# RohitMovva/VexAutonomousPlanner

Hardware: AMD Instinct MI355X
Metric: trajectory sample-points/sec (batched paths) (higher is better)
Workload: dtype f32; 1 GPU; c3: 4096 paths x 32 waypoints x 10000 samples per GPU; waypoints=32, samples=10000, recurrence=f64 behind fp32 rows, parallelism=paths sharded x1, no data-path collective

## Files before the change

### include/vap.h

```cpp
#ifndef VAP_H
#define VAP_H

#include <stddef.h>
#include <stdint.h>

#ifdef __cplusplus
extern "C" {
#endif

#define VAP_VERSION 100

typedef enum {
    VAP_OK = 0,
    VAP_ERR_INVALID = -1,
    VAP_ERR_NO_DEVICE = -2,
    VAP_ERR_HIP = -3,
    VAP_ERR_UNFITTED = -4,
    VAP_ERR_CAPACITY = -5,
    VAP_ERR_UNSUPPORTED = -6
} vap_status;

typedef enum { VAP_F32 = 0, VAP_F64 = 1 } vap_dtype;

typedef struct {
// ... 10 lines not shown
#define VAP_LUT_SAMPLES 1000
#define VAP_SAMPLES_PER_NODE 1000

typedef struct vap_ctx vap_ctx;

int vap_version(void);
const char *vap_status_string(int status);
const char *vap_last_error(void);
int vap_device_count(void);
int vap_ctx_create(int device, vap_ctx **out);
int vap_ctx_destroy(vap_ctx *ctx);
#define VAP_STREAM_OWN ((void *)(intptr_t)-1)
int vap_ctx_set_stream(vap_ctx *ctx, void *hip_stream);
int vap_ctx_synchronize(vap_ctx *ctx);
enum { VAP_OPT_VELOCITY_KERNEL = 0, VAP_OPT_F32_RECURRENCE = 1,
       VAP_OPT_TIME_DOMAIN_RESIDUAL = 3, VAP_OPT_TIME_KERNEL = 4, VAP_OPT_FOOTPRINT_CULL = 5 };
enum { VAP_VELOCITY_AUTO = 0, VAP_VELOCITY_SEQ_LITERAL = 1, VAP_VELOCITY_SEQ_FAST = 2, VAP_VELOCITY_RELAX = 3,
       VAP_VELOCITY_RELAX_BLOCK = 4 , VAP_VELOCITY_RELAX_WAVE = 5 ,
       VAP_VELOCITY_LANES = 6 , VAP_VELOCITY_LANES_16 = 7, VAP_VELOCITY_LANES_32 = 8,
       VAP_VELOCITY_LANES_64 = 9, VAP_VELOCITY_RELAX_ROUNDS = 10  };
enum { VAP_RECURRENCE_F64 = 0, VAP_RECURRENCE_F32 = 1 };
enum { VAP_TIME_KERNEL_AUTO = 0, VAP_TIME_KERNEL_LANE = 1, VAP_TIME_KERNEL_QUAD = 2, VAP_TIME_KERNEL_FUSED = 3 };
int vap_ctx_set_option(vap_ctx *ctx, int option, int value);
int vap_ctx_set_timing(vap_ctx *ctx, int enabled);
int vap_last_timing(vap_ctx *ctx, float ms[VAP_T_COUNT]);


int vap_fit(vap_ctx *ctx, vap_dtype dt, int B, int W, const void *d_waypoints,
            const double *d_tangent_in, const double *d_tangent_out, double *d_segments,
            double *d_segment_lengths , double *d_meta,
            uint32_t *d_flags);

int vap_fit_ex(vap_ctx *ctx, vap_dtype dt, int B, int W, const void *d_waypoints,
               const double *d_tangent_in, const double *d_tangent_out, const double *d_first_derivatives,
               const double *d_second_derivatives, const double *d_starting_tangent,
               const double *d_ending_tangent, double *d_segments, double *d_segment_lengths,
               double *d_first_out, double *d_second_out, double *d_meta, uint32_t *d_flags);
// ... 136 lines not shown
```

### vexautonomousplanner_amd/_lib.py

```python
import ctypes as C
import os

HERE = os.path.dirname(os.path.abspath(__file__))
LIB_PATH = os.path.join(HERE, "libvap.so")

VAP_OK = 0
VAP_ERR_INVALID = -1
VAP_ERR_NO_DEVICE = -2
VAP_ERR_HIP = -3
VAP_ERR_UNFITTED = -4
VAP_ERR_CAPACITY = -5
VAP_ERR_UNSUPPORTED = -6
VAP_F32 = 0
VAP_F64 = 1
FLAG_DEGENERATE = 1
FLAG_TRUNCATED = 2
FLAG_NOCONVERGE = 4
FLAG_BAD_ROUTE = 8
T_FIT, T_LUT, T_SAMPLE, T_VELOCITY, T_TOTAL, T_COUNT = 0, 1, 2, 3, 4, 8
OPT_VELOCITY_KERNEL = 0
OPT_TIME_DOMAIN_RESIDUAL = 3
OPT_F32_RECURRENCE = 1
OPT_TIME_KERNEL = 4
OPT_FOOTPRINT_CULL = 5
TIME_KERNEL_AUTO, TIME_KERNEL_LANE, TIME_KERNEL_QUAD, TIME_KERNEL_FUSED = 0, 1, 2, 3
RECURRENCE_F64, RECURRENCE_F32 = 0, 1
VELOCITY_AUTO, VELOCITY_SEQ_LITERAL, VELOCITY_SEQ_FAST, VELOCITY_RELAX = 0, 1, 2, 3
VELOCITY_RELAX_BLOCK, VELOCITY_RELAX_WAVE = 4, 5
VELOCITY_LANES, VELOCITY_LANES_16, VELOCITY_LANES_32, VELOCITY_LANES_64 = 6, 7, 8, 9
VELOCITY_RELAX_ROUNDS = 10
LUT_SAMPLES = 1000
SAMPLES_PER_NODE = 1000
CLOSEST_GUI, CLOSEST_EXACT = 0, 1
CLOSEST_MODES = {"gui": CLOSEST_GUI, "exact": CLOSEST_EXACT}


def closest_mode(mode):
    if mode in (CLOSEST_GUI, CLOSEST_EXACT) and not isinstance(mode, bool):
        return int(mode)
# ... 193 lines not shown
```

### vexautonomousplanner_amd/batch.py

```python
import ctypes as C

import numpy as np
import torch

from . import _lib
from .synth import DEFAULT_CONSTRAINTS, END_VEL, START_VEL

FIELDS = ("x", "y", "heading", "curvature", "velocity")


def _torch_dtype(dtype):
    if dtype in ("f32", "fp32", torch.float32, np.float32, _lib.VAP_F32):
        return torch.float32, _lib.VAP_F32
    if dtype in ("f64", "fp64", torch.float64, np.float64, _lib.VAP_F64):
        return torch.float64, _lib.VAP_F64
    raise ValueError(f"unsupported dtype {dtype!r}")


class ProfileResult(dict):
    generation = None


class BatchedTrajectoryGenerator:

# ... 8 lines not shown
        self._L = _lib.lib()
        self.set_velocity_kernel(velocity_kernel)
        self.set_recurrence(recurrence)
        self.time_domain_residual = bool(time_domain_residual)
        self.ctx.set_option(_lib.OPT_TIME_DOMAIN_RESIDUAL, 1 if self.time_domain_residual else 0)
        self._generation = 0

    def set_recurrence(self, which):
        self.recurrence = {"f64": "f64", "f32": "f32", "fp64": "f64", "fp32": "f32"}[which]
        self.ctx.set_option(_lib.OPT_F32_RECURRENCE,
                            _lib.RECURRENCE_F64 if self.recurrence == "f64" else _lib.RECURRENCE_F32)

    def set_time_kernel(self, which):
        self.ctx.set_option(_lib.OPT_TIME_KERNEL, {"auto": _lib.TIME_KERNEL_AUTO, "lane": _lib.TIME_KERNEL_LANE,
                                                   "quad": _lib.TIME_KERNEL_QUAD, "fused": _lib.TIME_KERNEL_FUSED}[which])

    def set_velocity_kernel(self, which):
        table = {"auto": _lib.VELOCITY_AUTO, "seq_literal": _lib.VELOCITY_SEQ_LITERAL,
                 "seq_fast": _lib.VELOCITY_SEQ_FAST, "relax": _lib.VELOCITY_RELAX,
                 "relax_block": _lib.VELOCITY_RELAX_BLOCK, "relax_wave": _lib.VELOCITY_RELAX_WAVE,
                 "lanes": _lib.VELOCITY_LANES, "lanes16": _lib.VELOCITY_LANES_16, "lanes32": _lib.VELOCITY_LANES_32,
                 "lanes64": _lib.VELOCITY_LANES_64, "relax_rounds": _lib.VELOCITY_RELAX_ROUNDS}
        self.ctx.set_option(_lib.OPT_VELOCITY_KERNEL, table[which])

    def profile(self, waypoints, constraints=DEFAULT_CONSTRAINTS, samples=None, dd=None,
                start_vel=START_VEL, end_vel=END_VEL, want=FIELDS, out=None, capacity=None):
        if (samples is None) == (dd is None):
            raise ValueError("give exactly one of samples= or dd=")
        wp = waypoints
        if wp.device != self.device or wp.dtype != self.tdtype or wp.dim() != 3 or wp.shape[2] != 2:
# ... 289 lines not shown
```

### vexautonomousplanner_amd/csrc/vap_api.hip

```cpp
#include <cstdlib>
#include <cstring>

#include "vap_internal.h"
#include "vap_kernels.h"

namespace {
thread_local std::string g_last_error;
}

int vap_fail(int status, const char *fmt, ...)
{
    char buf[512];
    va_list ap;
    va_start(ap, fmt);
    vsnprintf(buf, sizeof(buf), fmt, ap);
    va_end(ap);
    g_last_error = buf;
    return status;
}

int vap_set_device(vap_ctx *ctx)
{
    if (!ctx) return vap_fail(VAP_ERR_INVALID, "null context");
    HIP_TRY(hipSetDevice(ctx->device));
// ... 232 lines not shown
        return VAP_OK;
    }
    if (option == VAP_OPT_TIME_DOMAIN_RESIDUAL && (value == 0 || value == 1)) {
        ctx->keep_residual = value;
        ctx->vres_for = nullptr;
        return VAP_OK;
    }
    if (option == VAP_OPT_TIME_KERNEL && value >= VAP_TIME_KERNEL_AUTO && value <= VAP_TIME_KERNEL_FUSED) {
        ctx->time_kernel = value;
        return VAP_OK;
    }
    if (option == VAP_OPT_FOOTPRINT_CULL && (value == 0 || value == 1)) {
        ctx->footprint_cull = value;
        return VAP_OK;
    }
    if (option == VAP_OPT_F32_RECURRENCE && (value == VAP_RECURRENCE_F64 || value == VAP_RECURRENCE_F32)) {
        ctx->f32_recurrence = value;
        ctx->rows_valid = false;
        return VAP_OK;
    }
    return vap_fail(VAP_ERR_INVALID, "unknown option %d / value %d", option, value);
}

int vap_ctx_set_timing(vap_ctx *ctx, int enabled)
{
    if (!ctx) return vap_fail(VAP_ERR_INVALID, "null context");
    ctx->timing = enabled != 0;
    return VAP_OK;
}

int vap_last_timing(vap_ctx *ctx, float ms[VAP_T_COUNT])
{
    VAP_TRY(vap_set_device(ctx));
    if (!ms) return vap_fail(VAP_ERR_INVALID, "null output");
    for (int i = 0; i < VAP_T_COUNT; i++) ms[i] = 0.f;
    if (!ctx->timing) return VAP_OK;
    HIP_TRY(hipEventSynchronize(ctx->ev[VAP_T_VELOCITY + 1]));
    float total = 0.f;
    for (int i = 0; i <= VAP_T_VELOCITY; i++) {
        float t = 0.f;
        HIP_TRY(hipEventElapsedTime(&t, ctx->ev[i], ctx->ev[i + 1]));
        ms[i] = t;
        total += t;
    }
    ms[VAP_T_TOTAL] = total;
    return VAP_OK;
}

int vap_fit(vap_ctx *ctx, vap_dtype dt, int B, int W, const void *d_waypoints, const double *d_tangent_in,
            const double *d_tangent_out, double *d_segments, double *d_segment_lengths, double *d_meta,
            uint32_t *d_flags)
{
    VAP_TRY(vap_set_device(ctx));
    VAP_TRY(check_shape(B, W, 2));
    if (!d_waypoints || !d_segments || !d_meta) return vap_fail(VAP_ERR_INVALID, "null buffer");
    HIP_TRY(vap::launch_fit(ctx->stream, dt == VAP_F64, B, W, d_waypoints, d_tangent_in, d_tangent_out,
                            d_segments, nullptr, d_segment_lengths, d_meta, d_flags));
    return VAP_OK;
// ... 139 lines not shown
        VAP_TRY(ctx->ensure(ctx->flags, (size_t)B * sizeof(uint32_t)));
        flags = (uint32_t *)ctx->flags.ptr;
    }
    void *curv = d_curvature;
    if (!curv && !hi) {
        VAP_TRY(ctx->ensure(ctx->io[7], n_pts * esz(dt)));
        curv = ctx->io[7].ptr;
    }
    const double cc[6] = {c->max_vel, c->max_acc, c->max_acc, c->friction_coef, c->max_jerk, c->track_width};
    StageTimer tm(ctx);
    vap::GridArgs grid;
    grid.S = S;
    grid.dd = dd;
    grid.aux = (double *)ctx->aux.ptr;
    grid.runs = (double *)ctx->runs.ptr;
    if (vap::fit_lut_fusable(B, W)) {
        tm.mark(VAP_T_FIT);
        HIP_TRY(vap::launch_fit_lut(ctx->stream, f64, B, W, d_waypoints, (double *)ctx->seg.ptr, (double *)ctx->power.ptr,
                                    (double *)ctx->lut.ptr, meta, flags, grid));
    } else {
        HIP_TRY(vap::launch_fit(ctx->stream, f64, B, W, d_waypoints, nullptr, nullptr, (double *)ctx->seg.ptr,
                                (double *)ctx->power.ptr, nullptr, meta, flags));
        tm.mark(VAP_T_FIT);
        HIP_TRY(vap::launch_lut(ctx->stream, B, W, (const double *)ctx->seg.ptr, (double *)ctx->lut.ptr,
                                nullptr, meta, flags, grid));
    }
    tm.mark(VAP_T_LUT);
    {
        HIP_TRY(vap::launch_sample(ctx->stream, f64, B, W, S, (const double *)ctx->power.ptr, (const double *)ctx->lut.ptr, nullptr,
                                   meta, (const double *)ctx->aux.ptr, (const double *)ctx->runs.ptr, d_x, d_y, d_heading,
                                   curv, hi ? nullptr : ctx->dth.ptr, hi ? (double *)ctx->k64.ptr : nullptr,
                                   hi ? (double *)ctx->dth64.ptr : nullptr, (const double *)ctx->seg.ptr));
        tm.mark(VAP_T_SAMPLE);
        if (hi)
            VAP_TRY(run_velocity(ctx, true, false, B, S, cc, start_vel, end_vel, meta, ctx->k64.ptr, ctx->dth64.ptr, nullptr,
                                 vap::AccRowsV(), d_velocity, flags));
        else
            VAP_TRY(run_velocity(ctx, f64, f64, B, S, cc, start_vel, end_vel, meta, curv, ctx->dth.ptr, nullptr, vap::AccRowsV(),
                                 d_velocity, flags));
    }
    tm.mark(VAP_T_VELOCITY);
    ctx->last_B = B;
    ctx->last_W = W;
    ctx->grid_B = B;
    ctx->grid_W = W;
    ctx->grid_S = S;
    ctx->rows_valid = true;
// ... 46 lines not shown
    }
    void *curv = d_curvature;
    if (!curv && !hi) {
        VAP_TRY(ctx->ensure(ctx->io[7], n_pts * esz(dt)));
        curv = ctx->io[7].ptr;
    }
    const double cc[6] = {c->max_vel, c->max_acc, c->max_acc, c->friction_coef, c->max_jerk, c->track_width};
    vap::RouteSplitInputs in;
    in.rev = d_node_reverse;
    in.turn = d_node_turn;
    in.tangent = d_node_tangent;
    in.mag = d_node_magnitudes;
    double *sptab = (double *)ctx->sptab.ptr;
    int *nspl = (int *)ctx->nspl.ptr;
    StageTimer tm(ctx);
    HIP_TRY(vap::launch_fit_routes(ctx->stream, f64, B, W, NS, d_waypoints, in, (double *)ctx->seg.ptr, (double *)ctx->power.ptr,
                                   nullptr, sptab, nspl, meta, flags));
    tm.mark(VAP_T_FIT);
    vap::RouteTables rt;
    rt.sptab = sptab;
    rt.nspl = nspl;
    rt.NS = NS;
    const bool single = NS == 1;
    HIP_TRY(vap::launch_lut(ctx->stream, B, W, (const double *)ctx->seg.ptr, (double *)ctx->lut.ptr, nullptr, meta, flags,
                            vap::GridArgs(), rt));
    HIP_TRY(vap::launch_route_offsets(ctx->stream, B, W, NS, S, dd, (const double *)ctx->lut.ptr, sptab, nspl, meta,
                                      (double *)ctx->aux.ptr, (double *)ctx->runs.ptr, flags));
    tm.mark(VAP_T_LUT);
    if (single)
        HIP_TRY(vap::launch_sample(ctx->stream, f64, B, W, S, (const double *)ctx->power.ptr, (const double *)ctx->lut.ptr,
// ... 298 lines not shown
```

### vexautonomousplanner_amd/csrc/vap_internal.h

```cpp
#pragma once
#include "../../include/vap.h"

#include <hip/hip_runtime.h>

#include <cstdarg>
#include <cstdio>
#include <string>

int vap_fail(int status, const char *fmt, ...);

#define HIP_TRY(expr)                                                                              \
    do {                                                                                           \
        hipError_t e_ = (expr);                                                                    \
        if (e_ != hipSuccess)                                                                      \
            return vap_fail(VAP_ERR_HIP, "%s failed: %s (%s:%d)", #expr, hipGetErrorString(e_), __FILE__, __LINE__); \
    } while (0)

#define VAP_TRY(expr)            \
    do {                         \
        int s_ = (expr);         \
        if (s_ != VAP_OK) return s_; \
    } while (0)

struct VapBuffer {
// ... 5 lines not shown
    int device = 0;
    hipStream_t own_stream = nullptr;
    hipStream_t stream = nullptr;
    bool timing = false;
    int velocity_kernel = 0;
    int f32_recurrence = 0;
    hipEvent_t ev[VAP_T_COUNT + 1] = {};
    float ms[VAP_T_COUNT] = {};
    VapBuffer seg, power, lut, slopes, aux, runs, meta, dth, flags, io[8], small_in, small_out, small_seg, small_lut;
    VapBuffer ufwd, lstate, lcount;
    VapBuffer vhi, vres;
    const void *vres_for = nullptr;
    int vres_B = 0, vres_S = 0;
    int keep_residual = 1;
    int time_kernel = 0;
    VapBuffer k64, dth64;
    VapBuffer sptab, nspl;
    int route_NS = 0;
    int last_B = 0, last_W = 0;
    int grid_B = 0, grid_W = 0, grid_S = 0;
    bool rows_valid = false, rows_hi = false;
    int rows_dt = 0;
    int footprint_cull = 1;
    VapBuffer scene;
    void *scene_host = nullptr;
    size_t scene_host_cap = 0;
    hipEvent_t scene_ev = nullptr;

    int ensure(VapBuffer &b, size_t bytes)
    {
// ... 16 lines not shown
```

### vexautonomousplanner_amd/csrc/vap_kernels.h

```cpp
#pragma once
#include <hip/hip_runtime.h>
#include <stdint.h>

namespace vap {

constexpr uint32_t VAP_FLAG_DEGENERATE_BIT = 1u;
constexpr uint32_t VAP_FLAG_TRUNCATED_BIT = 2u;
constexpr uint32_t VAP_FLAG_NOCONVERGE_BIT = 4u;

constexpr int kSampleThreads = 256;
constexpr int kSPT = 4;
constexpr int kSampleChunk = kSampleThreads * kSPT;
constexpr int kSampleTile = kSampleChunk - kSPT;
constexpr int kCoefBlockDoubles = 36;
constexpr int kGridRunBlockDoubles = 3 * 100;
constexpr int kLdsCoefSegments = 112;
constexpr int kMaxWaypoints = 2048;
constexpr int kMaxRouteWaypoints = 1500;

struct RouteTables {
    const double *sptab = nullptr;
    const int *nspl = nullptr;
    int NS = 1;
};
struct RouteSplitInputs {
    const int *rev = nullptr;
    const double *turn = nullptr;
    const double *tangent = nullptr;
    const double *mag = nullptr;
};
hipError_t launch_fit(hipStream_t st, bool f64, int B, int W, const void *wp, const double *tin,
// ... 9 lines not shown
hipError_t launch_lut(hipStream_t st, int B, int W, const double *seg, double *lut, double *slopes, double *meta,
                      uint32_t *flags, GridArgs grid = GridArgs(), RouteTables rt = RouteTables());
bool fit_lut_fusable(int B, int W);
hipError_t launch_fit_lut(hipStream_t st, bool f64, int B, int W, const void *wp, double *seg, double *pw, double *lut,
                          double *meta, uint32_t *flags, GridArgs grid);
hipError_t launch_fit_routes(hipStream_t st, bool f64, int B, int W, int NS, const void *wp, const RouteSplitInputs &in, double *seg,
                             double *pw, double *seglen, double *sptab, int *nspl, double *meta, uint32_t *flags);
hipError_t launch_route_offsets(hipStream_t st, int B, int W, int NS, int S, double dd, const double *lut, double *sptab,
                                const int *nspl, double *meta, double *aux, double *runs, uint32_t *flags);
hipError_t launch_sample_routes(hipStream_t st, bool f64, int B, int W, int NS, int S, const double *pw, const double *lut,
                                const double *sptab, const int *nspl, const double *meta, const double *aux, const double *runs,
                                void *x, void *y, void *h, void *k, void *dth, double *k64, double *dth64, const double *seg);
hipError_t launch_lut_slopes(hipStream_t st, int B, const double *lut, const double *meta, double *slopes);
hipError_t launch_grid(hipStream_t st, int B, int W, int S, double dd, double *meta, double *aux, double *runs,
                       uint32_t *flags);
hipError_t launch_sample(hipStream_t st, bool f64, int B, int W, int S, const double *pw, const double *lut,
                         const double *slopes, const double *meta, const double *aux, const double *runs, void *x,
                         void *y, void *h, void *k, void *dth, double *k64, double *dth64,
                         const double *seg);
struct AccRowsV {
    const void *fwd = nullptr;
    const void *bwd = nullptr;
    const void *dec = nullptr;
};
hipError_t launch_velocity_seq(hipStream_t st, bool r64, bool io64, bool fast, int B, int S, const double c[6], double sv,
                               double ev, const double *meta, const void *curv, const void *dth, const void *vcap,
                               const AccRowsV &acc, void *vel, void *usq);
int velocity_relax_max_samples(bool f64, bool limits = false);
int velocity_relax_acc_max_samples(bool f64);
hipError_t launch_velocity_relax(hipStream_t st, bool r64, bool io64, int B, int S, const double c[6], double sv, double ev,
                                 const double *meta, const void *curv, const void *dth, const void *vcap,
                                 const AccRowsV &acc, void *vel, uint32_t *flags, void *vhi = nullptr);
size_t velocity_long_state_bytes(bool f64, int B, int S);
size_t velocity_long_counter_bytes(bool f64, int B, int S);
// ... 65 lines not shown
```

### vexautonomousplanner_amd/csrc/vap_kernels.hip

```cpp
#include "vap_device.h"
#include "vap_kernels.h"

#include <cstdio>
#include <cstdlib>
#include <type_traits>
#include <vector>

namespace vap {

static_assert(kCoefBlockDoubles == kCoefDoubles, "scratch sizing and block layout disagree");
static_assert(kGridRunBlockDoubles == kGridRunDoubles, "scratch sizing and run-table layout disagree");

struct FitExtras {
    const double *first = nullptr, *second = nullptr;
    const double *start_tan = nullptr, *end_tan = nullptr;
    double *out_first = nullptr, *out_second = nullptr;
};

template <typename IT>
__device__ __forceinline__ void fit_path(int b, int W, const IT *__restrict__ waypoints, const double *__restrict__ tan_in,
                                         const double *__restrict__ tan_out, const FitExtras &ex, double *__restrict__ segments,
                                         double *__restrict__ power, double *__restrict__ seglen, double *__restrict__ meta,
                                         uint32_t *__restrict__ flags, double *sh, int tid = threadIdx.x, int nt = blockDim.x,
                                         uint32_t *flag_word = nullptr)
// ... 134 lines not shown
    int b = blockIdx.x * per + sub;
    b = b < B ? b : B - 1;
    fit_path<IT>(b, W, waypoints, nullptr, nullptr, FitExtras(), segments, power, nullptr, meta, flags, sh + (size_t)sub * 7 * W, lane, L,
                 &s_flags[sub]);
}

__global__ void k_grid(int B, int W, int S, double dd_in, double *__restrict__ meta, double *__restrict__ aux,
                       double *__restrict__ runs, uint32_t *__restrict__ flags)
{
    const int b = blockIdx.x * blockDim.x + threadIdx.x;
    if (b >= B) return;
    grid_define(b, W, S, dd_in, meta[(size_t)b * kMetaStride + 1], meta[(size_t)b * kMetaStride + 0], meta, aux, runs, flags);
}

constexpr int kLutPad = (kLutN + 31) / 32 * 32;
template <bool SEG_LDS>
__device__ __forceinline__ void lut_path(int W, const double *__restrict__ segments, double *__restrict__ lut,
                                         double *__restrict__ slopes, double *__restrict__ meta, uint32_t *__restrict__ flags,
                                         const GridArgs &grid, const RouteTables &rt, long long *__restrict__ stats, double *s_seg,
                                         double *cum)
{
    const long long tl0 = stats ? __builtin_amdgcn_s_memtime() : 0;
    constexpr int kPad = kLutPad;
    double *mag = cum;
    const int b = blockIdx.x, tid = threadIdx.x, nt = blockDim.x;
    int G = W - 1;
    double t_max;
    const double *seg = segments + (size_t)b * (W - 1) * 12;
    size_t row = (size_t)b;
    if (rt.sptab) {
// ... 32 lines not shown
        for (int it = 0; it < kPer; it++) {
            const int j = tid + it * nt;
            inc[it] = (j > 0 && j < kLutN) ? (mag[j - 1] + mag[j]) * 0.5 * dt : 0.0;
        }
        __syncthreads();
#pragma unroll
        for (int it = 0; it < kPer; it++) {
            const int j = tid + it * nt;
            if (j < kPad) cum[j] = inc[it];
        }
    }
    __syncthreads();
    __shared__ double s_start[kPad / 32];
    __shared__ double s_total;
    if (tid == 0) {
        double acc = 0.0;
        const double2 *cum2 = reinterpret_cast<const double2 *>(cum);
#pragma unroll 1
        for (int g0 = 0; g0 < kPad / 32; g0++) {
            s_start[g0] = acc;
            double2 v[16];
#pragma unroll
            for (int k = 0; k < 16; k++) v[k] = cum2[g0 * 16 + k];
#pragma unroll
            for (int k = 0; k < 16; k++) { acc += v[k].x; acc += v[k].y; }
        }
        if (!rt.sptab) meta[(size_t)b * kMetaStride + 1] = acc;
        s_total = acc;
        if (flags && !(acc > 0.0 && isfinite(acc))) atomicOr(&flags[b], VAP_FLAG_DEGENERATE_BIT);
    }
    __syncthreads();
    if (grid.aux && !rt.sptab && tid == nt - 1) grid_define(b, W, grid.S, grid.dd, s_total, t_max, meta, grid.aux, grid.runs, flags);
    if (tid < kPad / 32) {
        double acc = s_start[tid];
        double2 *cum2 = reinterpret_cast<double2 *>(cum) + tid * 16;
        double2 v[16];
#pragma unroll
        for (int k = 0; k < 16; k++) v[k] = cum2[k];
#pragma unroll
        for (int k = 0; k < 16; k++) {
            acc += v[k].x;
            v[k].x = acc;
            acc += v[k].y;
            v[k].y = acc;
        }
#pragma unroll
        for (int k = 0; k < 16; k++) cum2[k] = v[k];
    }
    __syncthreads();
    const long long tl2 = stats ? __builtin_amdgcn_s_memtime() : 0;
    const double lstep = t_max / (double)(kLutN - 1);
    for (int j = tid; j < kLutN; j += nt) {
        lut[row * kLutN + j] = cum[j];
        if (slopes) {
            double w = 0.0;
            if (j > 0) {
                const double t0 = (double)(j - 1) * lstep, t1 = (j == kLutN - 1) ? t_max : (double)j * lstep;
                w = div_inrange(t1 - t0, cum[j] - cum[j - 1]);
            }
            slopes[row * kLutN + j] = w;
        }
    }
    if (stats && tid == 0) {
// ... 169 lines not shown
                             double *__restrict__ slopes)
{
    const int i = blockIdx.x * blockDim.x + threadIdx.x;
    if (i >= B * kLutN) return;
    const int b = i / kLutN, j = i % kLutN;
    const double t_max = meta[(size_t)b * kMetaStride + 0];
    const double lstep = t_max / (double)(kLutN - 1);
    double w = 0.0;
    if (j > 0) {
        const double t0 = (double)(j - 1) * lstep, t1 = (j == kLutN - 1) ? t_max : (double)j * lstep;
        w = div_inrange(t1 - t0, lut[i] - lut[i - 1]);
    }
    slopes[i] = w;
}

template <typename OT, bool COEF_LDS, bool HI, int PPB = 1>
__global__ __launch_bounds__(kSampleThreads, 3) void k_sample(int B, int W, int S, int tile, int tiles_per_block,
                                                           const double *__restrict__ power,
                                                           const double *__restrict__ seg_rows,
                                                           const double *__restrict__ lut,
                                                           const double *__restrict__ slopes,
                                                           const double *__restrict__ meta,
                                                           const double *__restrict__ aux,
                                                           const double *__restrict__ runs,
                                                           OT *__restrict__ ox, OT *__restrict__ oy,
                                                           OT *__restrict__ oh, OT *__restrict__ ok,
                                                           OT *__restrict__ odth, double *__restrict__ ok64,
                                                           double *__restrict__ odth64, long long *__restrict__ stats)
{
    static_assert(!HI || sizeof(OT) == 4, "the fp64 side rows belong to the fp32 output mode");
    extern __shared__ __attribute__((aligned(16))) double s_coef[];
    __shared__ double sD_all[PPB * kLutN], sWt_all[PPB * kLutN];
    __shared__ double s_dx[2][kSampleThreads], s_dy[2][kSampleThreads];
    __shared__ int s_j[2][kSampleThreads];
    __shared__ OT s_th[2][kSampleThreads];
    const long long ts0 = stats ? __builtin_amdgcn_s_memtime() : 0;
    const int tid = threadIdx.x;
    const int G = W - 1;
    const int tile0 = blockIdx.x * tiles_per_block;
    if (tile0 * tile >= S) return;
    const bool writer = tile == kSampleChunk || tid < kSampleThreads - 1;
    constexpr int VW = 16 / sizeof(OT);
    const bool aligned = (S % VW) == 0;

    int p_b[PPB], p_N[PPB], p_nruns[PPB];
    bool p_live[PPB];
    double p_tmax[PPB], p_total[PPB], p_dd[PPB], p_lstep[PPB], p_tstep[PPB], p_inv[PPB], p_sk[PPB];
    double run_touch = 0.0;
#pragma unroll
    for (int pp = 0; pp < PPB; pp++) {
        const int bq = blockIdx.y * PPB + pp;
        p_live[pp] = bq < B;
        const int b = p_live[pp] ? bq : B - 1;
        p_b[pp] = b;
        const double *m = meta + (size_t)b * kMetaStride;
        p_tmax[pp] = m[0]; p_total[pp] = m[1]; p_dd[pp] = m[2];
        p_N[pp] = (int)m[3];
        const double *ax = aux + (size_t)b * kAuxStride;
        p_lstep[pp] = ax[0]; p_tstep[pp] = ax[1]; p_inv[pp] = ax[2];
        p_nruns[pp] = (int)ax[3];
        run_touch += runs[(size_t)b * kGridRunDoubles + (tid < 120 ? tid : 0)];
    }
    __shared__ double s_end[PPB][2];
    double end_d1x = 1.0, end_d1y = 1.0;
    {
        const int pp = tid < PPB ? tid : 0;
        if (seg_rows && tid < PPB && p_live[pp]) {
            end_d1x = seg_rows[((size_t)p_b[pp] * G + (G - 1)) * 12 + 6];
            end_d1y = seg_rows[((size_t)p_b[pp] * G + (G - 1)) * 12 + 7];
        }
    }
    {
        constexpr int ITER = 4;
        double vD[PPB][ITER], vW[PPB][ITER];
#pragma unroll
        for (int pp = 0; pp < PPB; pp++) {
            const bool go = p_live[pp];
#pragma unroll
// ... 20 lines not shown
                if (p_live[pp])
                    lds_fill<4>(s_coef + (size_t)pp * G * kCoefDoubles, power + (size_t)p_b[pp] * G * kCoefDoubles, G * kCoefDoubles, tid,
                                kSampleThreads);
        }
#pragma unroll
        for (int pp = 0; pp < PPB; pp++) {
#pragma unroll
            for (int it = 0; it < ITER; it++) {
                const int i = tid + it * kSampleThreads;
                if (i < kLutN) {
                    sD_all[pp * kLutN + i] = vD[pp][it];
                    if (slopes) sWt_all[pp * kLutN + i] = vW[pp][it];
                }
            }
        }
    }
    auto grid_first_of = [&](const double *run_tab, double dd, int N, int n_runs, int kb0) {
        const int dd_exp = (__double2hiint(dd) >> 20) & 0x7ff;
        const int kf = kb0 < N - 1 ? kb0 : N - 1;
        int r = 2 + 2 * (((__double2hiint((double)kf * dd) >> 20) & 0x7ff) - dd_exp);
        r = kf <= 0 ? 0 : r < 1 ? 1 : r;
        r = r > n_runs - 1 ? n_runs - 1 : r;
        const double *e = run_tab + 3 * r;
        int ka = (int)grid_run_k0(e, 0);
        const int kb = (int)grid_run_k0(e, 1);
        double sa = e[1], da = e[2];
        if (kf < ka || kf >= kb) {
            while ((int)grid_run_k0(run_tab, r + 1) <= kf) r++;
            while (r > 0 && (int)grid_run_k0(run_tab, r) > kf) r--;
            ka = (int)grid_run_k0(run_tab, r);
            sa = run_tab[3 * r + 1];
            da = run_tab[3 * r + 2];
        }
        return sa + (double)(kf - ka) * da;
    };
#pragma unroll
    for (int pp = 0; pp < PPB; pp++)
        p_sk[pp] = (p_live[pp] && tile0 * tile < p_N[pp])
                       ? grid_first_of(runs + (size_t)p_b[pp] * kGridRunDoubles, p_dd[pp], p_N[pp], p_nruns[pp], tile0 * tile + tid * kSPT)
                       : 0.0;
    constexpr bool kSlopeOnDemand = PPB == 2;
    if (!slopes && !kSlopeOnDemand) {
        __syncthreads();
#pragma unroll
        for (int pp = 0; pp < PPB; pp++) {
            if (p_live[pp] && tile0 * tile < p_N[pp]) {
                const double *sDp = sD_all + pp * kLutN;
                for (int j = tid; j < kLutN; j += kSampleThreads) {
                    double w = 0.0;
                    if (j > 0) {
                        const double t0 = (double)(j - 1) * p_lstep[pp], t1 = (j == kLutN - 1) ? p_tmax[pp] : (double)j * p_lstep[pp];
                        w = div_inrange(t1 - t0, sDp[j] - sDp[j - 1]);
                    }
                    sWt_all[pp * kLutN + j] = w;
                }
            }
        }
    }
    __syncthreads();
    asm volatile("" ::"v"(run_touch));
    const long long ts1 = stats ? __builtin_amdgcn_s_memtime() : 0;
    const double end_param = (double)(W - 1);
    const int tab_n = W * kSamplesPerNode;
    int tiles_done = 0;

#pragma unroll 1
    for (int pp = 0; pp < PPB; pp++) {
    const int bq = blockIdx.y * PPB + pp;
    if (bq >= B) break;
    const int b = bq;
    const double *m = meta + (size_t)b * kMetaStride;
    const double t_max = m[0], total = m[1], dd = m[2];
    const int N = (int)m[3];
    const double *ax = aux + (size_t)b * kAuxStride;
    const double lstep = ax[0], tstep = ax[1], inv_tstep = ax[2];
    const int n_runs = (int)ax[3];
    const size_t row = (size_t)b * S;
    const double *sD = sD_all + pp * kLutN, *sWt = sWt_all + pp * kLutN;
    const double *pw = power + (size_t)b * G * kCoefDoubles;
    const double *coef = COEF_LDS ? s_coef + (size_t)pp * G * kCoefDoubles : pw;
    const double *run_tab = runs + (size_t)b * kGridRunDoubles;
    const double sk_first = PPB == 1 ? p_sk[0] : (pp == 0 ? p_sk[0] : p_sk[PPB - 1]);
    auto grid_first = [&](int kb0) { return grid_first_of(run_tab, dd, N, n_runs, kb0); };
    for (int tl = 0; tl < tiles_per_block; tl++) {
        const int k0 = (tile0 + tl) * tile;
        if (k0 >= S) break;
        const int kbase = k0 + tid * kSPT;
        auto store_vec = [&](OT *dst, const OT v[kSPT]) {
            if (!dst || !writer) return;
            if (aligned && kbase + kSPT <= S) {
                if constexpr (sizeof(OT) == 4) {
                    if constexpr (HI) {
                        using f4 = float __attribute__((ext_vector_type(4)));
                        f4 w = {v[0], v[1], v[2], v[3]};
                        __builtin_nontemporal_store(w, reinterpret_cast<f4 *>(dst + row + kbase));
                    } else {
// ... 235 lines not shown
            }
            store_vec(ox, vx); store_vec(oy, vy); store_vec(oh, vh); store_vec(ok, vk);
            if constexpr (HI) store_hi(odth64, vd64);
            store_vec(odth, vd);
        }
            };
        const bool interior = k0 > 0 && k0 + kSampleThreads * kSPT < N - 1 && aligned && (S & 1) == 0 && k0 + kSampleThreads * kSPT <= S;
        if (interior) tile_body(std::true_type{});
        else tile_body(std::false_type{});
    }
    }
    if (stats && (tid & 63) == 0) {
        long long *st = stats + ((size_t)(blockIdx.y * gridDim.x + blockIdx.x) * 4 + (tid >> 6)) * 4;
        st[0] = ts1 - ts0;
        st[1] = __builtin_amdgcn_s_memtime() - ts1;
        st[2] = 0;
        st[3] = 0;
    }
}


template <typename R, typename IO, bool FAST>
__global__ __launch_bounds__(64) void k_velocity_seq(int B, int S, VelConsts<R> c, R start_u, R end_u,
                                                     const double *__restrict__ meta,
                                                     const R *__restrict__ curv, const R *__restrict__ dtheta,
                                                     const R *__restrict__ vcap, AccRows<R> acc, IO *__restrict__ vel,
                                                     R *__restrict__ usq)
{
    const int b = blockIdx.x * blockDim.x + threadIdx.x;
    if (b >= B) return;
    const double *m = meta + (size_t)b * kMetaStride;
    const R twodd = (R)2 * (R)m[2];
// ... 1371 lines not shown
}

hipError_t launch_lut_slopes(hipStream_t st, int B, const double *lut, const double *meta, double *slopes)
{
    hipLaunchKernelGGL(k_lut_slopes, dim3((B * kLutN + 255) / 256), dim3(256), 0, st, B, lut, meta, slopes);
    return hipGetLastError();
}

hipError_t launch_grid(hipStream_t st, int B, int W, int S, double dd, double *meta, double *aux, double *runs,
                       uint32_t *flags)
{
    hipLaunchKernelGGL(k_grid, dim3((B + 63) / 64), dim3(64), 0, st, B, W, S, dd, meta, aux, runs, flags);
    return hipGetLastError();
}

hipError_t launch_sample(hipStream_t st, bool f64, int B, int W, int S, const double *pw, const double *lut,
                         const double *slopes, const double *meta, const double *aux, const double *runs, void *x,
                         void *y, void *h, void *k, void *dth, double *k64, double *dth64, const double *seg)
{
    const bool hi = !f64 && k64 && dth64;
    const int tile = S <= kSampleChunk ? kSampleChunk : kSampleTile;
    const int n_tiles = (S + tile - 1) / tile;
    int split = (2048 + B - 1) / B;
    split = split < 1 ? 1 : (split > n_tiles ? n_tiles : split);
    const int tiles_per_block = (n_tiles + split - 1) / split;
    const bool in_lds = (W - 1) <= kLdsCoefSegments;
    const int ppb = (n_tiles == 1 && B >= 8192 && in_lds && (W - 1) <= 16) ? 2 : 1;
    const dim3 grid((n_tiles + tiles_per_block - 1) / tiles_per_block, (B + ppb - 1) / ppb);
    const size_t lds = in_lds ? sizeof(double) * (size_t)ppb * (W - 1) * kCoefDoubles : 0;
    static const bool want_stats = getenv("VAP_SAMPLE_STATS") != nullptr;
    long long *stats = nullptr;
    const size_t n_waves = (size_t)grid.x * grid.y * 4;
    if (want_stats) (void)hipMalloc(&stats, n_waves * 4 * sizeof(long long));
#define VAP_SAMPLE(OT_, LDS_, HI_, PPB_)                                                                            \
    hipLaunchKernelGGL((k_sample<OT_, LDS_, HI_, PPB_>), grid, dim3(kSampleThreads), lds, st, B, W, S, tile, tiles_per_block, pw, seg, lut, \
                       slopes, meta, aux, runs, (OT_ *)x, (OT_ *)y, (OT_ *)h, (OT_ *)k, (OT_ *)dth, k64, dth64, stats)
    if (ppb == 2) {
        if (f64) VAP_SAMPLE(double, true, false, 2);
        else if (hi) VAP_SAMPLE(float, true, true, 2);
        else VAP_SAMPLE(float, true, false, 2);
    } else if (f64) { if (in_lds) VAP_SAMPLE(double, true, false, 1); else VAP_SAMPLE(double, false, false, 1); }
    else if (hi) { if (in_lds) VAP_SAMPLE(float, true, true, 1); else VAP_SAMPLE(float, false, true, 1); }
    else { if (in_lds) VAP_SAMPLE(float, true, false, 1); else VAP_SAMPLE(float, false, false, 1); }
#undef VAP_SAMPLE
    if (stats) {
        std::vector<long long> h(n_waves * 4);
        (void)hipStreamSynchronize(st);
        (void)hipMemcpy(h.data(), stats, h.size() * sizeof(long long), hipMemcpyDeviceToHost);
        (void)hipFree(stats);
        double sum[4] = {0, 0, 0, 0};
        for (size_t w = 0; w < n_waves; w++)
            for (int k = 0; k < 4; k++) sum[k] += (double)h[w * 4 + k];
        fprintf(stderr, "[sample grid %ux%u, %d tiles/block] per-wave mean ticks: stage %.0f tiles %.0f\n", grid.x,
                grid.y, tiles_per_block, sum[0] / n_waves, sum[1] / n_waves);
    }
    return hipGetLastError();
}

template <typename R>
static VelConsts<R> make_consts(const double c[6])
{
    VelConsts<R> v;
    v.vmax = (R)c[0];
    v.amax = (R)c[1];
    v.adec = (R)c[2];
    v.tw = (R)c[5];
    v.wmax = (R)2 * v.vmax / v.tw;
// ... 348 lines not shown
```

Measured before the change: 46.42 billion sample-points/s.

## Fuse spline fit and arc-length LUT build into the sampling kernel

Adds a FIT variant of the sample kernel in which each workgroup fits its own path's spline, builds the arc-length table and grid runs in LDS, and then samples directly. The separate fit/LUT launch and the global round trip of coefficients, LUT, meta and aux are removed, though the results are still written back to global memory for later stages. On by default when B>=2048, W-1<=48 and one path per block. The cost is serial fit work at the start of every sampling workgroup, higher LDS use that may lower occupancy, and wider template specialisation.

```diff
diff --git a/include/vap.h b/include/vap.h
--- a/include/vap.h
+++ b/include/vap.h
@@ -48,13 +48,14 @@
 int vap_ctx_set_stream(vap_ctx *ctx, void *hip_stream);
 int vap_ctx_synchronize(vap_ctx *ctx);
 enum { VAP_OPT_VELOCITY_KERNEL = 0, VAP_OPT_F32_RECURRENCE = 1,
-       VAP_OPT_TIME_DOMAIN_RESIDUAL = 3, VAP_OPT_TIME_KERNEL = 4, VAP_OPT_FOOTPRINT_CULL = 5 };
+       VAP_OPT_TIME_DOMAIN_RESIDUAL = 3, VAP_OPT_TIME_KERNEL = 4, VAP_OPT_FOOTPRINT_CULL = 5, VAP_OPT_FIT_IN_SAMPLER = 6 };
 enum { VAP_VELOCITY_AUTO = 0, VAP_VELOCITY_SEQ_LITERAL = 1, VAP_VELOCITY_SEQ_FAST = 2, VAP_VELOCITY_RELAX = 3,
        VAP_VELOCITY_RELAX_BLOCK = 4 , VAP_VELOCITY_RELAX_WAVE = 5 ,
        VAP_VELOCITY_LANES = 6 , VAP_VELOCITY_LANES_16 = 7, VAP_VELOCITY_LANES_32 = 8,
        VAP_VELOCITY_LANES_64 = 9, VAP_VELOCITY_RELAX_ROUNDS = 10  };
 enum { VAP_RECURRENCE_F64 = 0, VAP_RECURRENCE_F32 = 1 };
 enum { VAP_TIME_KERNEL_AUTO = 0, VAP_TIME_KERNEL_LANE = 1, VAP_TIME_KERNEL_QUAD = 2, VAP_TIME_KERNEL_FUSED = 3 };
+enum { VAP_FIT_IN_SAMPLER_AUTO = 0, VAP_FIT_IN_SAMPLER_OFF = 1 };
 int vap_ctx_set_option(vap_ctx *ctx, int option, int value);
 int vap_ctx_set_timing(vap_ctx *ctx, int enabled);
 int vap_last_timing(vap_ctx *ctx, float ms[VAP_T_COUNT]);
diff --git a/vexautonomousplanner_amd/_lib.py b/vexautonomousplanner_amd/_lib.py
--- a/vexautonomousplanner_amd/_lib.py
+++ b/vexautonomousplanner_amd/_lib.py
@@ -23,6 +23,8 @@
 OPT_F32_RECURRENCE = 1
 OPT_TIME_KERNEL = 4
 OPT_FOOTPRINT_CULL = 5
+OPT_FIT_IN_SAMPLER = 6
+FIT_IN_SAMPLER_AUTO, FIT_IN_SAMPLER_OFF = 0, 1
 TIME_KERNEL_AUTO, TIME_KERNEL_LANE, TIME_KERNEL_QUAD, TIME_KERNEL_FUSED = 0, 1, 2, 3
 RECURRENCE_F64, RECURRENCE_F32 = 0, 1
 VELOCITY_AUTO, VELOCITY_SEQ_LITERAL, VELOCITY_SEQ_FAST, VELOCITY_RELAX = 0, 1, 2, 3
diff --git a/vexautonomousplanner_amd/batch.py b/vexautonomousplanner_amd/batch.py
--- a/vexautonomousplanner_amd/batch.py
+++ b/vexautonomousplanner_amd/batch.py
@@ -46,6 +46,9 @@
     def set_time_kernel(self, which):
         self.ctx.set_option(_lib.OPT_TIME_KERNEL, {"auto": _lib.TIME_KERNEL_AUTO, "lane": _lib.TIME_KERNEL_LANE,
                                                    "quad": _lib.TIME_KERNEL_QUAD, "fused": _lib.TIME_KERNEL_FUSED}[which])
+
+    def set_fit_in_sampler(self, which):
+        self.ctx.set_option(_lib.OPT_FIT_IN_SAMPLER, {"auto": _lib.FIT_IN_SAMPLER_AUTO, "off": _lib.FIT_IN_SAMPLER_OFF}[which])
 
     def set_velocity_kernel(self, which):
         table = {"auto": _lib.VELOCITY_AUTO, "seq_literal": _lib.VELOCITY_SEQ_LITERAL,
diff --git a/vexautonomousplanner_amd/csrc/vap_api.hip b/vexautonomousplanner_amd/csrc/vap_api.hip
--- a/vexautonomousplanner_amd/csrc/vap_api.hip
+++ b/vexautonomousplanner_amd/csrc/vap_api.hip
@@ -270,6 +270,10 @@
         ctx->footprint_cull = value;
         return VAP_OK;
     }
+    if (option == VAP_OPT_FIT_IN_SAMPLER && (value == VAP_FIT_IN_SAMPLER_AUTO || value == VAP_FIT_IN_SAMPLER_OFF)) {
+        ctx->fit_in_sampler = value;
+        return VAP_OK;
+    }
     if (option == VAP_OPT_F32_RECURRENCE && (value == VAP_RECURRENCE_F64 || value == VAP_RECURRENCE_F32)) {
         ctx->f32_recurrence = value;
         ctx->rows_valid = false;
@@ -298,6 +302,10 @@
         HIP_TRY(hipEventElapsedTime(&t, ctx->ev[i], ctx->ev[i + 1]));
         ms[i] = t;
         total += t;
+    }
+    if (ctx->timed_fit_in_sampler) {
+        ms[VAP_T_SAMPLE] += ms[VAP_T_FIT] + ms[VAP_T_LUT];
+        ms[VAP_T_FIT] = ms[VAP_T_LUT] = 0.f;
     }
     ms[VAP_T_TOTAL] = total;
     return VAP_OK;
@@ -467,7 +475,21 @@
     grid.dd = dd;
     grid.aux = (double *)ctx->aux.ptr;
     grid.runs = (double *)ctx->runs.ptr;
-    if (vap::fit_lut_fusable(B, W)) {
+    const bool fit_in_sampler = ctx->fit_in_sampler == VAP_FIT_IN_SAMPLER_AUTO && vap::sample_fit_fusable(B, W, S);
+    vap::SampleFitArgs<true> sfit;
+    sfit.waypoints = d_waypoints;
+    sfit.dd = dd;
+    sfit.seg = (double *)ctx->seg.ptr;
+    sfit.power = (double *)ctx->power.ptr;
+    sfit.lut = (double *)ctx->lut.ptr;
+    sfit.meta = meta;
+    sfit.aux = (double *)ctx->aux.ptr;
+    sfit.runs = (double *)ctx->runs.ptr;
+    sfit.flags = flags;
+    if (ctx->timing) ctx->timed_fit_in_sampler = fit_in_sampler;
+    if (fit_in_sampler) {
+        tm.mark(VAP_T_FIT);
+    } else if (vap::fit_lut_fusable(B, W)) {
         tm.mark(VAP_T_FIT);
         HIP_TRY(vap::launch_fit_lut(ctx->stream, f64, B, W, d_waypoints, (double *)ctx->seg.ptr, (double *)ctx->power.ptr,
                                     (double *)ctx->lut.ptr, meta, flags, grid));
@@ -483,7 +505,8 @@
         HIP_TRY(vap::launch_sample(ctx->stream, f64, B, W, S, (const double *)ctx->power.ptr, (const double *)ctx->lut.ptr, nullptr,
                                    meta, (const double *)ctx->aux.ptr, (const double *)ctx->runs.ptr, d_x, d_y, d_heading,
                                    curv, hi ? nullptr : ctx->dth.ptr, hi ? (double *)ctx->k64.ptr : nullptr,
-                                   hi ? (double *)ctx->dth64.ptr : nullptr, (const double *)ctx->seg.ptr));
+                                   hi ? (double *)ctx->dth64.ptr : nullptr, (const double *)ctx->seg.ptr,
+                                   fit_in_sampler ? &sfit : nullptr));
         tm.mark(VAP_T_SAMPLE);
         if (hi)
             VAP_TRY(run_velocity(ctx, true, false, B, S, cc, start_vel, end_vel, meta, ctx->k64.ptr, ctx->dth64.ptr, nullptr,
@@ -560,6 +583,7 @@
     double *sptab = (double *)ctx->sptab.ptr;
     int *nspl = (int *)ctx->nspl.ptr;
     StageTimer tm(ctx);
+    if (ctx->timing) ctx->timed_fit_in_sampler = false;
     HIP_TRY(vap::launch_fit_routes(ctx->stream, f64, B, W, NS, d_waypoints, in, (double *)ctx->seg.ptr, (double *)ctx->power.ptr,
                                    nullptr, sptab, nspl, meta, flags));
     tm.mark(VAP_T_FIT);
diff --git a/vexautonomousplanner_amd/csrc/vap_internal.h b/vexautonomousplanner_amd/csrc/vap_internal.h
--- a/vexautonomousplanner_amd/csrc/vap_internal.h
+++ b/vexautonomousplanner_amd/csrc/vap_internal.h
@@ -43,6 +43,8 @@
     int vres_B = 0, vres_S = 0;
     int keep_residual = 1;
     int time_kernel = 0;
+    int fit_in_sampler = 0;
+    bool timed_fit_in_sampler = false;
     VapBuffer k64, dth64;
     VapBuffer sptab, nspl;
     int route_NS = 0;
diff --git a/vexautonomousplanner_amd/csrc/vap_kernels.h b/vexautonomousplanner_amd/csrc/vap_kernels.h
--- a/vexautonomousplanner_amd/csrc/vap_kernels.h
+++ b/vexautonomousplanner_amd/csrc/vap_kernels.h
@@ -15,6 +15,8 @@
 constexpr int kCoefBlockDoubles = 36;
 constexpr int kGridRunBlockDoubles = 3 * 100;
 constexpr int kLdsCoefSegments = 112;
+constexpr int kFitLdsSegments = 48;
+constexpr int kFitMinPaths = 2048;
 constexpr int kMaxWaypoints = 2048;
 constexpr int kMaxRouteWaypoints = 1500;
 
@@ -54,10 +56,21 @@
 hipError_t launch_lut_slopes(hipStream_t st, int B, const double *lut, const double *meta, double *slopes);
 hipError_t launch_grid(hipStream_t st, int B, int W, int S, double dd, double *meta, double *aux, double *runs,
                        uint32_t *flags);
+template <bool FIT>
+struct SampleFitArgs {};
+template <>
+struct SampleFitArgs<true> {
+    const void *waypoints = nullptr;
+    double dd = 0.0;
+    double *seg = nullptr, *power = nullptr, *lut = nullptr, *meta = nullptr, *aux = nullptr, *runs = nullptr;
+    uint32_t *flags = nullptr;
+};
+bool sample_fit_fusable(int B, int W, int S);
 hipError_t launch_sample(hipStream_t st, bool f64, int B, int W, int S, const double *pw, const double *lut,
                          const double *slopes, const double *meta, const double *aux, const double *runs, void *x,
                          void *y, void *h, void *k, void *dth, double *k64, double *dth64,
-                         const double *seg);
+                         const double *seg,
+                         const SampleFitArgs<true> *fit = nullptr);
 struct AccRowsV {
     const void *fwd = nullptr;
     const void *bwd = nullptr;
diff --git a/vexautonomousplanner_amd/csrc/vap_kernels.hip b/vexautonomousplanner_amd/csrc/vap_kernels.hip
--- a/vexautonomousplanner_amd/csrc/vap_kernels.hip
+++ b/vexautonomousplanner_amd/csrc/vap_kernels.hip
@@ -172,6 +172,38 @@
 }
 
 constexpr int kLutPad = (kLutN + 31) / 32 * 32;
+__device__ __forceinline__ double lut_chain_walk(const double *cum, double *s_start)
+{
+    double acc = 0.0;
+    const double2 *cum2 = reinterpret_cast<const double2 *>(cum);
+#pragma unroll 1
+    for (int g0 = 0; g0 < kLutPad / 32; g0++) {
+        s_start[g0] = acc;
+        double2 v[16];
+#pragma unroll
+        for (int k = 0; k < 16; k++) v[k] = cum2[g0 * 16 + k];
+#pragma unroll
+        for (int k = 0; k < 16; k++) { acc += v[k].x; acc += v[k].y; }
+    }
+    return acc;
+}
+__device__ __forceinline__ void lut_chain_replay(double *cum, const double *s_start, int g)
+{
+    double acc = s_start[g];
+    double2 *cum2 = reinterpret_cast<double2 *>(cum) + g * 16;
+    double2 v[16];
+#pragma unroll
+    for (int k = 0; k < 16; k++) v[k] = cum2[k];
+#pragma unroll
+    for (int k = 0; k < 16; k++) {
+        acc += v[k].x;
+        v[k].x = acc;
+        acc += v[k].y;
+        v[k].y = acc;
+    }
+#pragma unroll
+    for (int k = 0; k < 16; k++) cum2[k] = v[k];
+}
 template <bool SEG_LDS>
 __device__ __forceinline__ void lut_path(int W, const double *__restrict__ segments, double *__restrict__ lut,
                                          double *__restrict__ slopes, double *__restrict__ meta, uint32_t *__restrict__ flags,
@@ -234,39 +266,14 @@
     __shared__ double s_start[kPad / 32];
     __shared__ double s_total;
     if (tid == 0) {
-        double acc = 0.0;
-        const double2 *cum2 = reinterpret_cast<const double2 *>(cum);
-#pragma unroll 1
-        for (int g0 = 0; g0 < kPad / 32; g0++) {
-            s_start[g0] = acc;
-            double2 v[16];
-#pragma unroll
-            for (int k = 0; k < 16; k++) v[k] = cum2[g0 * 16 + k];
-#pragma unroll
-            for (int k = 0; k < 16; k++) { acc += v[k].x; acc += v[k].y; }
-        }
+        const double acc = lut_chain_walk(cum, s_start);
         if (!rt.sptab) meta[(size_t)b * kMetaStride + 1] = acc;
         s_total = acc;
         if (flags && !(acc > 0.0 && isfinite(acc))) atomicOr(&flags[b], VAP_FLAG_DEGENERATE_BIT);
     }
     __syncthreads();
     if (grid.aux && !rt.sptab && tid == nt - 1) grid_define(b, W, grid.S, grid.dd, s_total, t_max, meta, grid.aux, grid.runs, flags);
-    if (tid < kPad / 32) {
-        double acc = s_start[tid];
-        double2 *cum2 = reinterpret_cast<double2 *>(cum) + tid * 16;
-        double2 v[16];
-#pragma unroll
-        for (int k = 0; k < 16; k++) v[k] = cum2[k];
-#pragma unroll
-        for (int k = 0; k < 16; k++) {
-            acc += v[k].x;
-            v[k].x = acc;
-            acc += v[k].y;
-            v[k].y = acc;
-        }
-#pragma unroll
-        for (int k = 0; k < 16; k++) cum2[k] = v[k];
-    }
+    if (tid < kPad / 32) lut_chain_replay(cum, s_start, tid);
     __syncthreads();
     const long long tl2 = stats ? __builtin_amdgcn_s_memtime() : 0;
     const double lstep = t_max / (double)(kLutN - 1);
@@ -466,7 +473,14 @@
     slopes[i] = w;
 }
 
-template <typename OT, bool COEF_LDS, bool HI, int PPB = 1>
+template <bool UNIFORM>
+__device__ __forceinline__ double path_scalar(const double *p)
+{
+    const double v = *p;
+    if constexpr (!UNIFORM) return v;
+    return __hiloint2double(__builtin_amdgcn_readfirstlane(__double2hiint(v)), __builtin_amdgcn_readfirstlane(__double2loint(v)));
+}
+template <typename OT, bool COEF_LDS, bool HI, int PPB = 1, bool FIT = false>
 __global__ __launch_bounds__(kSampleThreads, 3) void k_sample(int B, int W, int S, int tile, int tiles_per_block,
                                                            const double *__restrict__ power,
                                                            const double *__restrict__ seg_rows,
@@ -478,11 +492,14 @@
                                                            OT *__restrict__ ox, OT *__restrict__ oy,
                                                            OT *__restrict__ oh, OT *__restrict__ ok,
                                                            OT *__restrict__ odth, double *__restrict__ ok64,
-                                                           double *__restrict__ odth64, long long *__restrict__ stats)
+                                                           double *__restrict__ odth64, long long *__restrict__ stats,
+                                                           SampleFitArgs<FIT> fit)
 {
     static_assert(!HI || sizeof(OT) == 4, "the fp64 side rows belong to the fp32 output mode");
+    static_assert(!FIT || (PPB == 1 && COEF_LDS), "the fitting workgroup owns one path and keeps its blocks in LDS");
     extern __shared__ __attribute__((aligned(16))) double s_coef[];
-    __shared__ double sD_all[PPB * kLutN], sWt_all[PPB * kLutN];
+    constexpr int kTabDoubles = FIT ? kLutPad : PPB * kLutN;
+    __shared__ __attribute__((aligned(FIT ? 16 : 8))) double sD_all[kTabDoubles], sWt_all[kTabDoubles];
     __shared__ double s_dx[2][kSampleThreads], s_dy[2][kSampleThreads];
     __shared__ int s_j[2][kSampleThreads];
     __shared__ OT s_th[2][kSampleThreads];
@@ -499,6 +516,70 @@
     bool p_live[PPB];
     double p_tmax[PPB], p_total[PPB], p_dd[PPB], p_lstep[PPB], p_tstep[PPB], p_inv[PPB], p_sk[PPB];
     double run_touch = 0.0;
+    __shared__ double s_end[PPB][2];
+    double *f_meta = nullptr, *f_aux = nullptr, *f_runs = nullptr;
+    uint32_t *f_flag = nullptr;
+    if constexpr (FIT) {
+        __shared__ double fs_meta[kMetaStride], fs_aux[kAuxStride], fs_runs[kGridRunDoubles], fs_start[kLutPad / 32];
+        __shared__ uint32_t fs_flag;
+        f_meta = fs_meta; f_aux = fs_aux; f_runs = fs_runs; f_flag = &fs_flag;
+        const int b = blockIdx.y;
+        double *s_seg = s_coef + (size_t)G * kCoefDoubles;
+        fit_path<OT>(0, W, (const OT *)fit.waypoints + (size_t)b * W * 2, nullptr, nullptr, FitExtras(), s_seg, s_coef, nullptr, fs_meta,
+                     &fs_flag, sWt_all);
+        __syncthreads();
+        if (stats && (tid & 63) == 0)
+            stats[((size_t)(blockIdx.y * gridDim.x + blockIdx.x) * 4 + (tid >> 6)) * 4 + 2] = __builtin_amdgcn_s_memtime() - ts0;
+        const double t_max = fs_meta[0];
+        const double step = t_max / (double)(kLutN - 1);
+#pragma unroll 1
+        for (int j = tid; j < kLutPad; j += kSampleThreads) {
+            double mg = 0.0;
+            if (j < kLutN) {
+                const double t = (j == kLutN - 1) ? t_max : (double)j * step;
+                double lt, dx, dy;
+                int idx;
+                normalize_parameter(t, t_max, G, lt, idx);
+                hermite_d1_ref(s_seg + (size_t)idx * 12, lt, dx, dy);
+                mg = sqrt(dx * dx + dy * dy);
+            }
+            sWt_all[j] = mg;
+        }
+        __syncthreads();
+        const double dt = (double)1 * step - (double)0 * step;
+#pragma unroll 1
+        for (int j = tid; j < kLutPad; j += kSampleThreads)
+            sD_all[j] = (j > 0 && j < kLutN) ? (sWt_all[j - 1] + sWt_all[j]) * 0.5 * dt : 0.0;
+        __syncthreads();
+        const bool chain_wave = __builtin_amdgcn_readfirstlane(tid) == 0;
+        if (chain_wave) __builtin_amdgcn_s_setprio(3);
+        if (tid == 0) {
+            const double acc = lut_chain_walk(sD_all, fs_start);
+            fs_meta[1] = acc;
+            if (!(acc > 0.0 && isfinite(acc))) atomicOr(&fs_flag, VAP_FLAG_DEGENERATE_BIT);
+        }
+        if (chain_wave) __builtin_amdgcn_s_setprio(0);
+        __syncthreads();
+        if (tid == kSampleThreads - 1) grid_define(0, W, S, fit.dd, fs_meta[1], t_max, fs_meta, fs_aux, fs_runs, &fs_flag);
+        if (tid < kLutPad / 32) lut_chain_replay(sD_all, fs_start, tid);
+        __syncthreads();
+        if (stats && (tid & 63) == 0)
+            stats[((size_t)(blockIdx.y * gridDim.x + blockIdx.x) * 4 + (tid >> 6)) * 4 + 3] = __builtin_amdgcn_s_memtime() - ts0;
+        p_live[0] = true;
+        p_b[0] = b;
+        p_tmax[0] = fs_meta[0]; p_total[0] = fs_meta[1]; p_dd[0] = fs_meta[2];
+        p_N[0] = (int)fs_meta[3];
+        p_lstep[0] = fs_aux[0]; p_tstep[0] = fs_aux[1]; p_inv[0] = fs_aux[2];
+        p_nruns[0] = (int)fs_aux[3];
+        if (tid == 0) {
+            const double end_d1x = s_seg[(size_t)(G - 1) * 12 + 6], end_d1y = s_seg[(size_t)(G - 1) * 12 + 7];
+            double rx = 1.0, ry = 1.0;
+            if (fabs(end_d1x) <= 1e-9 * fabs(end_d1y) || fabs(end_d1y) <= 1e-9 * fabs(end_d1x))
+                hermite_eval_ref(s_seg, p_tmax[0], G, 1, (double)(W - 1), rx, ry);
+            s_end[0][0] = fabs(rx) <= 1e-12 * fabs(ry) ? rx : __builtin_nan("");
+            s_end[0][1] = fabs(ry) <= 1e-12 * fabs(rx) ? ry : __builtin_nan("");
+        }
+    } else {
 #pragma unroll
     for (int pp = 0; pp < PPB; pp++) {
         const int bq = blockIdx.y * PPB + pp;
@@ -513,7 +594,6 @@
         p_nruns[pp] = (int)ax[3];
         run_touch += runs[(size_t)b * kGridRunDoubles + (tid < 120 ? tid : 0)];
     }
-    __shared__ double s_end[PPB][2];
     double end_d1x = 1.0, end_d1y = 1.0;
     {
         const int pp = tid < PPB ? tid : 0;
@@ -564,6 +644,7 @@
                 }
             }
         }
+    }
     }
     auto grid_first_of = [&](const double *run_tab, double dd, int N, int n_runs, int kb0) {
         const int dd_exp = (__double2hiint(dd) >> 20) & 0x7ff;
@@ -587,7 +668,7 @@
 #pragma unroll
     for (int pp = 0; pp < PPB; pp++)
         p_sk[pp] = (p_live[pp] && tile0 * tile < p_N[pp])
-                       ? grid_first_of(runs + (size_t)p_b[pp] * kGridRunDoubles, p_dd[pp], p_N[pp], p_nruns[pp], tile0 * tile + tid * kSPT)
+                       ? grid_first_of(FIT ? f_runs : runs + (size_t)p_b[pp] * kGridRunDoubles, p_dd[pp], p_N[pp], p_nruns[pp], tile0 * tile + tid * kSPT)
                        : 0.0;
     constexpr bool kSlopeOnDemand = PPB == 2;
     if (!slopes && !kSlopeOnDemand) {
@@ -608,7 +689,21 @@
         }
     }
     __syncthreads();
-    asm volatile("" ::"v"(run_touch));
+    if constexpr (FIT) {
+        const size_t b = (size_t)p_b[0];
+        auto put2 = [&](double *dst, const double *src, int n) {
+            for (int i = tid; i < n / 2; i += kSampleThreads) reinterpret_cast<double2 *>(dst)[i] = reinterpret_cast<const double2 *>(src)[i];
+        };
+        put2(fit.seg + b * G * 12, s_coef + (size_t)G * kCoefDoubles, G * 12);
+        put2(fit.power + b * G * kCoefDoubles, s_coef, G * kCoefDoubles);
+        put2(fit.lut + b * kLutN, sD_all, kLutN);
+        for (int i = tid; i < 3 * (p_nruns[0] + 4); i += kSampleThreads) fit.runs[b * kGridRunDoubles + i] = f_runs[i];
+        if (tid < kMetaStride) fit.meta[b * kMetaStride + tid] = f_meta[tid];
+        else if (tid < kMetaStride + kAuxStride) fit.aux[b * kAuxStride + tid - kMetaStride] = f_aux[tid - kMetaStride];
+        if (tid == 64) fit.flags[b] = *f_flag;
+    } else {
+        asm volatile("" ::"v"(run_touch));
+    }
     const long long ts1 = stats ? __builtin_amdgcn_s_memtime() : 0;
     const double end_param = (double)(W - 1);
     const int tab_n = W * kSamplesPerNode;
@@ -619,17 +714,17 @@
     const int bq = blockIdx.y * PPB + pp;
     if (bq >= B) break;
     const int b = bq;
-    const double *m = meta + (size_t)b * kMetaStride;
-    const double t_max = m[0], total = m[1], dd = m[2];
-    const int N = (int)m[3];
-    const double *ax = aux + (size_t)b * kAuxStride;
-    const double lstep = ax[0], tstep = ax[1], inv_tstep = ax[2];
-    const int n_runs = (int)ax[3];
+    const double *m = FIT ? f_meta : meta + (size_t)b * kMetaStride;
+    const double t_max = path_scalar<FIT>(m + 0), total = path_scalar<FIT>(m + 1), dd = path_scalar<FIT>(m + 2);
+    const int N = (int)path_scalar<FIT>(m + 3);
+    const double *ax = FIT ? f_aux : aux + (size_t)b * kAuxStride;
+    const double lstep = path_scalar<FIT>(ax + 0), tstep = path_scalar<FIT>(ax + 1), inv_tstep = path_scalar<FIT>(ax + 2);
+    const int n_runs = (int)path_scalar<FIT>(ax + 3);
     const size_t row = (size_t)b * S;
     const double *sD = sD_all + pp * kLutN, *sWt = sWt_all + pp * kLutN;
     const double *pw = power + (size_t)b * G * kCoefDoubles;
     const double *coef = COEF_LDS ? s_coef + (size_t)pp * G * kCoefDoubles : pw;
-    const double *run_tab = runs + (size_t)b * kGridRunDoubles;
+    const double *run_tab = FIT ? f_runs : runs + (size_t)b * kGridRunDoubles;
     const double sk_first = PPB == 1 ? p_sk[0] : (pp == 0 ? p_sk[0] : p_sk[PPB - 1]);
     auto grid_first = [&](int kb0) { return grid_first_of(run_tab, dd, N, n_runs, kb0); };
     for (int tl = 0; tl < tiles_per_block; tl++) {
@@ -895,8 +990,10 @@
         long long *st = stats + ((size_t)(blockIdx.y * gridDim.x + blockIdx.x) * 4 + (tid >> 6)) * 4;
         st[0] = ts1 - ts0;
         st[1] = __builtin_amdgcn_s_memtime() - ts1;
-        st[2] = 0;
-        st[3] = 0;
+        if constexpr (!FIT) {
+            st[2] = 0;
+            st[3] = 0;
+        }
     }
 }
 
@@ -2298,9 +2395,23 @@
     return hipGetLastError();
 }
 
+static int sample_paths_per_block(int B, int W, int S)
+{
+    const int tile = S <= kSampleChunk ? kSampleChunk : kSampleTile;
+    const int n_tiles = (S + tile - 1) / tile;
+    return (n_tiles == 1 && B >= 8192 && (W - 1) <= kLdsCoefSegments && (W - 1) <= 16) ? 2 : 1;
+}
+
+bool sample_fit_fusable(int B, int W, int S)
+{
+    return fit_lut_fusable(B, W) && B >= kFitMinPaths && sample_paths_per_block(B, W, S) == 1 && (W - 1) <= kFitLdsSegments &&
+           (W - 1) <= kLdsCoefSegments;
+}
+
 hipError_t launch_sample(hipStream_t st, bool f64, int B, int W, int S, const double *pw, const double *lut,
                          const double *slopes, const double *meta, const double *aux, const double *runs, void *x,
-                         void *y, void *h, void *k, void *dth, double *k64, double *dth64, const double *seg)
+                         void *y, void *h, void *k, void *dth, double *k64, double *dth64, const double *seg,
+                         const SampleFitArgs<true> *fit)
 {
     const bool hi = !f64 && k64 && dth64;
     const int tile = S <= kSampleChunk ? kSampleChunk : kSampleTile;
@@ -2309,7 +2420,7 @@
     split = split < 1 ? 1 : (split > n_tiles ? n_tiles : split);
     const int tiles_per_block = (n_tiles + split - 1) / split;
     const bool in_lds = (W - 1) <= kLdsCoefSegments;
-    const int ppb = (n_tiles == 1 && B >= 8192 && in_lds && (W - 1) <= 16) ? 2 : 1;
+    const int ppb = sample_paths_per_block(B, W, S);
     const dim3 grid((n_tiles + tiles_per_block - 1) / tiles_per_block, (B + ppb - 1) / ppb);
     const size_t lds = in_lds ? sizeof(double) * (size_t)ppb * (W - 1) * kCoefDoubles : 0;
     static const bool want_stats = getenv("VAP_SAMPLE_STATS") != nullptr;
@@ -2318,8 +2429,17 @@
     if (want_stats) (void)hipMalloc(&stats, n_waves * 4 * sizeof(long long));
 #define VAP_SAMPLE(OT_, LDS_, HI_, PPB_)                                                                            \
     hipLaunchKernelGGL((k_sample<OT_, LDS_, HI_, PPB_>), grid, dim3(kSampleThreads), lds, st, B, W, S, tile, tiles_per_block, pw, seg, lut, \
-                       slopes, meta, aux, runs, (OT_ *)x, (OT_ *)y, (OT_ *)h, (OT_ *)k, (OT_ *)dth, k64, dth64, stats)
-    if (ppb == 2) {
+                       slopes, meta, aux, runs, (OT_ *)x, (OT_ *)y, (OT_ *)h, (OT_ *)k, (OT_ *)dth, k64, dth64, stats, SampleFitArgs<false>())
+#define VAP_SAMPLE_FIT(OT_, HI_)                                                                                    \
+    hipLaunchKernelGGL((k_sample<OT_, true, HI_, 1, true>), grid, dim3(kSampleThreads), lds + sizeof(double) * (size_t)(W - 1) * 12, st, B, W, S, \
+                       tile, tiles_per_block, pw, seg, lut, slopes, meta, aux, runs, (OT_ *)x, (OT_ *)y, (OT_ *)h, (OT_ *)k, (OT_ *)dth, k64,  \
+                       dth64, stats, *fit)
+    if (fit) {
+        if (!sample_fit_fusable(B, W, S) || split != 1 || grid.x != 1 || slopes) return hipErrorInvalidValue;
+        if (f64) VAP_SAMPLE_FIT(double, false);
+        else if (hi) VAP_SAMPLE_FIT(float, true);
+        else VAP_SAMPLE_FIT(float, false);
+    } else if (ppb == 2) {
         if (f64) VAP_SAMPLE(double, true, false, 2);
         else if (hi) VAP_SAMPLE(float, true, true, 2);
         else VAP_SAMPLE(float, true, false, 2);
@@ -2327,6 +2447,7 @@
     else if (hi) { if (in_lds) VAP_SAMPLE(float, true, true, 1); else VAP_SAMPLE(float, false, true, 1); }
     else { if (in_lds) VAP_SAMPLE(float, true, false, 1); else VAP_SAMPLE(float, false, false, 1); }
 #undef VAP_SAMPLE
+#undef VAP_SAMPLE_FIT
     if (stats) {
         std::vector<long long> h(n_waves * 4);
         (void)hipStreamSynchronize(st);
@@ -2335,6 +2456,10 @@
         double sum[4] = {0, 0, 0, 0};
         for (size_t w = 0; w < n_waves; w++)
             for (int k = 0; k < 4; k++) sum[k] += (double)h[w * 4 + k];
+        if (fit)
+            fprintf(stderr, "[sample+fit grid %ux%u, %d tiles/block] per-wave mean ticks: stage %.0f (fit done at %.0f, table at %.0f) tiles %.0f\n",
+                    grid.x, grid.y, tiles_per_block, sum[0] / n_waves, sum[2] / n_waves, sum[3] / n_waves, sum[1] / n_waves);
+        else
         fprintf(stderr, "[sample grid %ux%u, %d tiles/block] per-wave mean ticks: stage %.0f tiles %.0f\n", grid.x,
                 grid.y, tiles_per_block, sum[0] / n_waves, sum[1] / n_waves);
     }
```

Measured after the change: 46.99 billion sample-points/s, median of 6. 1.2% higher.
